# ahuang73/HemoCell

Measured on AMD Instinct MI355X. Metric: MLUPS + cell-vertex updates/s, 256^3 pipeflow 10% Hct, higher is better.
Workload: dtype f64

## Files before the change

### hemocell_amd/capi.py

```python
import ctypes as C
import os
import subprocess

_HERE = os.path.dirname(os.path.abspath(__file__))
LIB_PATH = os.path.join(_HERE, "lib", "libhemocell_amd.so")

c_double_p = C.POINTER(C.c_double)
c_long_p = C.POINTER(C.c_long)
c_int_p = C.POINTER(C.c_int)


class HcError(RuntimeError):
    pass


class Params(C.Structure):
    _fields_ = [(n, C.c_double) for n in
                ("dx", "dt", "nu_p", "rho_p", "kBT_p", "tau", "nu_lbm", "dm", "df", "f_limit", "kBT_lbm")]


class Material(C.Structure):
    _fields_ = [("kLink", C.c_double), ("kArea", C.c_double), ("kVolume", C.c_double), ("kBend", C.c_double),
                ("eta_m", C.c_double), ("radius", C.c_double), ("min_triangles", C.c_int),
                ("aspect_ratio", C.c_double), ("inner_edges", c_long_p), ("n_inner", C.c_int)]
# ... 34 lines not shown
    "hcl_slab_refresh_halos": (C.c_int, [VP, C.c_int]),
    "hcp_slab_sync_placement": (C.c_int, [VP, c_long_p]),
    "hcp_set_envelope": (C.c_int, [VP, C.c_double, c_double_p]),
    "hcp_envelope": (C.c_int, [VP, c_double_p, c_long_p]),
    "hcp_set_deletion_mode": (C.c_int, [VP, C.c_int]),
    "hcp_delete_incomplete_cells": (C.c_int, [VP, c_long_p]),
    "hcp_deletion_counts": (C.c_int, [VP, c_long_p, c_long_p, c_long_p, c_long_p]),
    "hcp_download_alive": (C.c_int, [VP, VP]),
    "hc_profile_enable": (C.c_int, [C.c_int]),
    "hc_profile_read": (C.c_int, [C.c_char_p, c_double_p, c_long_p]),
    "hc_profile_reset": (C.c_int, []),
    "hc_build_tag": (C.c_char_p, []),
    "hc_measure_copy_bandwidth": (C.c_int, [C.c_size_t, C.c_int, c_double_p]),
    "hcl_node_counts": (C.c_int, [VP, c_long_p]),
    "hc_debug_ibm_per_vertex": (C.c_int, [C.c_int]),
    "hc_set_reproducible_spread": (C.c_int, [C.c_int]),
    "hc_debug_force_plane_padding": (C.c_int, [C.c_int]),
    "hcl_create": (C.c_int, [C.POINTER(VP), C.c_int, C.c_int, C.c_int, c_int_p, C.c_double, C.c_int, C.c_int, C.c_int]),
    "hcl_destroy": (C.c_int, [VP]),
    "hcl_set_mask": (C.c_int, [VP, VP]),
    "hcl_init_equilibrium": (C.c_int, [VP, C.c_double, c_double_p]),
    "hcl_set_body_force_regions": (C.c_int, [VP, C.c_int, C.POINTER(C.c_int), c_double_p]),
    "hcl_set_body_force": (C.c_int, [VP, c_double_p]),
    "hcl_set_wall_velocity": (C.c_int, [VP, C.c_int, c_double_p]),
    "hcl_collide_stream": (C.c_int, [VP, C.c_int]),
    "hcl_set_lees_edwards": (C.c_int, [VP, C.c_double, C.c_double]),
    "hcl_set_lees_edwards_displacement": (C.c_int, [VP, C.c_double, C.c_double]),
    "hcl_lees_edwards_apply": (C.c_int, [VP]),
    "hcl_lees_edwards_state": (C.c_int, [VP, c_double_p]),
    "hcl_open_boundary_add": (C.c_int, [VP, C.c_int, C.c_int, c_int_p, C.c_int, c_int_p]),
# ... 165 lines not shown
```

### hemocell_amd/csrc/cells.h

```cpp
#pragma once
#include "common.h"
#include "host_cells.h"
#include "mesh.h"
#include <algorithm>
#include <cmath>
#include <cstring>

using namespace hc;

struct hc_celltype {
  CellTables host;
  DevBuf<int> d_tri, d_edge, d_ebt, d_ebo, d_iedge, d_vtri, d_vtri_k, d_vedge, d_vedge_s, d_bsrc, d_vouter, d_vinner, d_vinner_s, d_ring, d_nring;
  DevBuf<double> d_tri_area_eq, d_edge_len_eq, d_edge_angle_eq, d_patch_eq, d_iedge_len_eq;
};

struct hc_cells {
  hc_lattice *L = nullptr;
  hc_params P;
  int ntypes = 0;
  hc_celltype *types[8];
  int timescale[8];
  HostCells host[8];
  bool host_dirty = false;
  long nverts = 0, cap = 0;
// ... 107 lines not shown
        if (ok) {
          weight = phi2(p[0] - (double)gx) * phi2(p[1] - (double)gy) * phi2(p[2] - (double)gz);
          if (weight != 0.0) {
            node = (lx + HALO) * (long)v.plane + ly * v.nz + lz;
            if (v.mask[node] != 0) node = -1;
          }
        }
        if (node >= 0) total += weight;
        s.node[idx] = node; s.w[idx] = weight; s.lx[idx] = (int)lx; s.ly[idx] = (int)ly; s.lz[idx] = (int)lz;
      }
  const double coeff = 1.0 / total;
#pragma unroll
  for (int idx = 0; idx < 8; idx++) s.w[idx] *= coeff;
}

struct VertArrays { double *p[3], *v[3], *f[3], *r[3]; unsigned char *dead; int *tag; };
struct TypeArrays : VertArrays { const int *vert_cell; int *tag_all; };

template <typename T>
inline int upload_vec(DevBuf<T> &dst, const std::vector<T> &src) {
  const int rc = dst.reserve(src.size() ? src.size() : 1); if (rc != HC_OK) return rc;
  if (src.size()) HC_HIP(hipMemcpy(dst, src.data(), src.size() * sizeof(T), hipMemcpyHostToDevice));
  return HC_OK;
}
template <size_t N>
inline std::vector<int> flatten(const std::vector<std::array<long, N>> &v) {
  std::vector<int> o; o.reserve(v.size() * N);
  for (auto &a : v) for (long x : a) o.push_back((int)x);
  return o;
}
// ... 4 lines not shown
TypeArrays vert_arrays(hc_cells *C, int t);
int ensure_sflag(hc_cells *C);
int solidify_refresh_mask(hc_cells *C);
int solidify_check(hc_cells *C);
const char *solidify_refusal(const hc_lattice *L);
int ensure_rep(hc_cells *C);
int stage_ints(hc_cells *C, int which, int **d, const int *h, int n);
int stage_ints(Staged<int> &s, int **d, const int *h, int n);
int upload_xyz(DevBuf<double> dst[3], long first, const double *src, long n);
int download_xyz(double *dst, const DevBuf<double> src[3], long first, long n);
int append_cells(hc_cells *C, int type, const long *cell_ids, const int *is_new, int n, long n_new);
int interpolate_cells_staged(hc_cells *C, int type, const int *slots, int n, int which);
int wide_spread(hc_cells *C, int type, int force_limit, int per_vertex);
int wide_interpolate(hc_cells *C, int type, const int *slots, int n, int per_vertex);
int wide_emit(hc_cells *C, int type, const int *d_order, long ebase, int force_limit);
inline int ibm_width(const hc_cells *C, int type) { return C->ibm_kernel[type]; }

}
using namespace hcc;
```

### hemocell_amd/csrc/cells.hip

```cpp
#include "cells.h"
#include <cstddef>
#include <memory>
#include <unordered_map>
#include <utility>
#include <vector>

namespace {

__global__ __launch_bounds__(256) void advance_kernel(LatView v, long n, double *px, double *py, double *pz, const double *vx,
                                                      const double *vy, const double *vz, const int *vert_cell, int *tag, unsigned char *dead,
                                                      int *counters, int whole_cell) {
  const long i = (long)blockIdx.x * 256 + threadIdx.x;
  if (i >= n) return;
  const int cell = vert_cell[i];
  if (dead[i] || tag[cell] == 1) return;
  const double x = px[i] + vx[i], y = py[i] + vy[i], z = pz[i] + vz[i];
  px[i] = x; py[i] = y; pz[i] = z;
  long gx = nearest_node(x) - v.x0, gy = nearest_node(y), gz = nearest_node(z);
  bool inside = true;
  if (v.wrap_x) gx = pmod(gx, v.nx); else inside = inside && (gx >= (v.halo_x ? -HALO : 0) && gx < (v.halo_x ? v.nx + HALO : v.nx));
  if (gy < 0 || gy >= v.ny) { if (v.per_y) gy = pmod(gy, v.ny); else inside = false; }
  if (gz < 0 || gz >= v.nz) { if (v.per_z) gz = pmod(gz, v.nz); else inside = false; }
  if (inside && v.mask[(gx + HALO) * (long)v.plane + gy * v.nz + gz] != 0) {
    if (whole_cell) {
      if (atomicExch(&tag[cell], 1) != 1) atomicAdd(&counters[0], 1);
    } else {
      dead[i] = 1;
      atomicAdd(&counters[2], 1);
      if (atomicCAS(&tag[cell], 0, 2) == 0) atomicAdd(&counters[1], 1);
    }
  }
}

__global__ void publish_counters_kernel(const int *counters, int *host_view) { for (int k = 0; k < 4; k++) host_view[k] = counters[k]; }
__global__ void sub_counters_kernel(int *counters, int a, int b, int c, int d) { atomicSub(&counters[0], a); atomicSub(&counters[1], b); atomicSub(&counters[2], c); if (d) atomicSub(&counters[3], d); }

__global__ void delete_incomplete_kernel(long ncells, int *tag, int *counters) {
  const long c = (long)blockIdx.x * 256 + threadIdx.x;
  if (c >= ncells) return;
  if (tag[c] == 2) { tag[c] = 1; atomicAdd(&counters[0], 1); }
}

__global__ void add_vertex_force_kernel(int n, const long *idx, const double *f, double *fx, double *fy, double *fz) {
  const int i = blockIdx.x * 256 + threadIdx.x;
  if (i >= n) return;
  const long v = idx[i];
// ... 668 lines not shown
  if (particles_removed) *particles_removed = C->n_particles_deleted;
  if (incomplete_cells) *incomplete_cells = inc;
  if (missing_particles) *missing_particles = miss;
  return HC_OK;
}

int hcp_download_alive(hc_cells *C, unsigned char *alive) {
  HC_REQUIRE(C && alive, "hcp_download_alive: null pointer");
  int rc = settle(C); if (rc != HC_OK) return rc;
  rc = sync_to_host(C); if (rc != HC_OK) return rc;
  size_t o = 0;
  for (int t = 0; t < C->ntypes; t++) for (unsigned char d : C->host[t].dead) alive[o++] = d ? 0 : 1;
  return HC_OK;
}

int hcp_advance(hc_cells *C, int check_deletions) {
  HC_REQUIRE(C, "hcp_advance: null pointer");
  int rc = sync_to_device(C); if (rc != HC_OK) return rc;
  if (C->nverts == 0) return HC_OK;
  {
    hc::ProfScope prof(hc::PK_ADVANCE);
    const LatView v = make_view(C->L);
    for (int t = 0; t < C->ntypes; t++) {
      const long n = C->ncells[t] * C->types[t]->host.nv;
      if (n == 0) continue;
      const TypeArrays a = vert_arrays(C, t);
      hipLaunchKernelGGL(advance_kernel, dim3((unsigned)((n + 255) / 256)), dim3(256), 0, hc::stream(), v, n, a.p[0], a.p[1], a.p[2], a.v[0], a.v[1], a.v[2],
                         a.vert_cell, a.tag_all, a.dead, C->d_ntag, C->del_mode == HC_DELETE_CELL ? 1 : 0);
      HC_HIP(hipGetLastError());
    }
    C->maybe_tagged = true;
  }
  if (check_deletions) return settle(C);
  return HC_OK;
}

static int g_overlap = 1;
static int g_spread_beside = 1;
int hc_set_overlap(int on) { g_overlap = on != 0; g_spread_beside = on != 2; hcs::set_overlap(on); return HC_OK; }

int hc_iterate(hc_lattice *L, hc_cells *C, long *iter, int n, int particle_timescale, int force_limit, int deletion_check_every) {
  HC_REQUIRE(L && C && iter, "hc_iterate: null pointer");
  HC_REQUIRE(C->L == L, "hc_iterate: cells are bound to a different lattice");
  HC_REQUIRE(particle_timescale >= 1 && deletion_check_every >= 1, "hc_iterate: timescales must be >= 1");
  if (L->n_slabs > 1) return hcs::iterate_slab(L, C, iter, n, particle_timescale, force_limit);
  const bool visc = C->visc_on();
  if (visc) HC_REQUIRE(C->visc_every % particle_timescale == 0 && C->visc_grid_every % particle_timescale == 0,
                       "hc_iterate: the velocity-update timescale must divide both interior-viscosity timescales (hcp_set_interior_timescales)");
  const bool solid = C->solidify_on();
  if (solid) { const char *why = solidify_refusal(L); if (why) { hc::set_error(std::string("hc_iterate: ") + why); return HC_ERR_STATE; } }
// ... 11 lines not shown
      if ((rc = hcp_spread(C, force_limit)) != HC_OK) return rc;
    }
    spread_done = false;
    const bool particle_step = it % particle_timescale == 0;
    const bool visc_grid = visc && it % C->visc_grid_every == 0, visc_membrane = visc && it % C->visc_every == 0;
    const bool solid_check = solid && it % C->solid_every == 0;
    const bool overlap = may_overlap && !particle_step && !visc_grid && !visc_membrane && !solid_check && s + 1 < n;
    if (overlap && (rc = hc::fork()) != HC_OK) return rc;
    if ((rc = hcl_collide_stream_part(L, 0)) != HC_OK) return rc;
    hcl_step_end(L);
    if (L->le_on) {
      if ((rc = hc::lees_edwards_step(L)) != HC_OK) return rc;
      if (L->le_d != 0.0) L->le_D = fmod(L->le_d * (double)(it + 1), (double)L->nx);
    }
    if (L->scalar && (rc = hcl_scalar_step(L->scalar)) != HC_OK) return rc;
    if (particle_step) { if ((rc = hcp_interpolate(C)) != HC_OK) return rc; }
    if (solid_check) { if ((rc = solidify_check(C)) != HC_OK) return rc; }
    if (overlap) hc::route(1);
    if ((rc = hcp_advance(C, 0)) != HC_OK) return rc;
    if ((rc = hcp_mechanics(C, it, 0)) != HC_OK) return rc;
    if (overlap) {
      if (g_spread_beside) { if ((rc = hcp_spread(C, force_limit)) != HC_OK) return rc; spread_done = true; }
      if ((rc = hc::join()) != HC_OK) return rc;
    }
    if (visc_grid) {
      if ((rc = hcp_delete_incomplete_cells(C, nullptr)) != HC_OK) return rc;
      if ((rc = hcp_interior_find(C)) != HC_OK) return rc;
    }
    if (visc_membrane) { if ((rc = hcp_interior_membrane(C)) != HC_OK) return rc; }
    *iter = it + 1;
    if (!overlap && (it + 1) % deletion_check_every == 0 && s + 1 < n) { if ((rc = poll_deletions(C, true)) != HC_OK) return rc; }
  }
  if ((rc = poll_deletions(C, true)) != HC_OK) return rc;
  return solid ? solidify_refresh_mask(C) : HC_OK;
}

}
// ... 1 lines not shown
```

### hemocell_amd/csrc/common.h

```cpp
#pragma once
#include <hip/hip_runtime.h>
#include <stdint.h>
#include <string>
#include <utility>
#include <vector>
#include <type_traits>
#include "../../include/hemocell_amd.h"
#include "d3q19.h"

namespace hc {

void set_error(const std::string &msg);
int hip_fail(hipError_t e, const char *what, const char *file, int line);
hipStream_t stream();
hipStream_t comm_stream();
int fork();
void route(int side);
int join();
bool forked();

#define HC_HIP(call)                                                         \
  do {                                                                       \
    hipError_t e__ = (call);                                                 \
    if (e__ != hipSuccess) return hc::hip_fail(e__, #call, __FILE__, __LINE__); \
// ... 54 lines not shown
  ~Event() { if (e) (void)hipEventDestroy(e); }
  operator hipEvent_t() const { return e; }
  int create() {
    if (e) return HC_OK;
    const hipError_t r = hipEventCreateWithFlags(&e, hipEventDisableTiming);
    if (r != hipSuccess) { e = nullptr; return hip_fail(r, "hipEventCreateWithFlags", __FILE__, __LINE__); }
    return HC_OK;
  }
};
template <class T> struct Staged {
  DevBuf<T> d; PinBuf<T> h; Event ev;
  size_t cap() const { return d.cap < h.cap ? d.cap : h.cap; }
  int reserve(size_t n) { const int rc = d.reserve(n); return rc != HC_OK ? rc : h.reserve(n); }
};

enum ProfKernel { PK_COLLIDE = 0, PK_SPREAD, PK_INTERP, PK_ADVANCE, PK_MECH, PK_COLLIDE_BESIDE, PK_LEES_EDWARDS, PK_COLLIDE_VISC, PK_INTERIOR_FIND, PK_INTERIOR_MEMBRANE, PK_SCALAR, PK_SOLIDIFY_PREPARE, PK_SOLIDIFY_FLAG, PK_COUNT };
void prof_count(int kernel);
struct ProfScope {
  int k; bool on;
  hipEvent_t a, b;
  explicit ProfScope(int kernel);
  ~ProfScope();
};

constexpr int HALO = 2;

constexpr int STAT_BLOCKS = 512;
struct StatAcc { double mn, mx, sum; long n; };
__device__ __forceinline__ void stat_add(StatAcc &a, double v) { a.mn = v < a.mn ? v : a.mn; a.mx = v > a.mx ? v : a.mx; a.sum += v; a.n++; }
__device__ __forceinline__ void stat_block_store(StatAcc a, double *partial ) {
  __shared__ double s_red[4][4];
// ... 167 lines not shown
```

### hemocell_amd/csrc/ibm.hip

```cpp
#include "ibm_common.h"
#include <hipcub/hipcub.hpp>
#include <cstdlib>
#include <cstring>
#include <numeric>

namespace {

__global__ __launch_bounds__(256) void ibm_spread_kernel(LatView v, long n, const double *px, const double *py, const double *pz,
                                                         double *fx, double *fy, double *fz, const double *rx, const double *ry, const double *rz,
                                                         double *F, int limit_on, double f_limit, const int *vert_cell, const int *tag, const unsigned char *dead) {
  const long i = (long)blockIdx.x * 256 + threadIdx.x;
  if (i >= n) return;
  if (dead[i] || tag[vert_cell[i]] == 1) return;
  double f0 = fx[i], f1 = fy[i], f2 = fz[i];
  if (limit_on) {
    const double mag = sqrt((f0 * f0 + f1 * f1) + f2 * f2);
    if (mag > f_limit) {
      const double sc = f_limit / mag;
      f0 *= sc; f1 *= sc; f2 *= sc;
      fx[i] = f0; fy[i] = f1; fz[i] = f2;
    }
  }
  Stencil s;
  phi2_stencil(v, px[i], py[i], pz[i], s);
// ... 170 lines not shown
  if (nb[0] * nb[1] * nb[2] > 64) return false;
  if (threadIdx.x < 64) {
    const int l = threadIdx.x;
    bool near = false;
    if (l < nb[0] * nb[1] * nb[2]) {
      const int bz = l % nb[2], by = (l / nb[2]) % nb[1], bx = l / (nb[2] * nb[1]);
      near = v.wallbrick[((long)(b0[0] + bx) * v.nby + (b0[1] + by)) * v.nbz + (b0[2] + bz)] != 0;
    }
    const unsigned long long any = __ballot(near);
    if (l == 0) *s_near = any != 0ull;
  }
  __syncthreads();
  return *s_near == 0;
}

__device__ __forceinline__ bool cell_prologue(const LatView &v, int nv, long base, const double *px, const double *py, const double *pz,
                                              const unsigned char *dead, int *s_red, int *s_near, unsigned char *mt, Tile &t, VStencil vs[NVPT] PH_PARAM) {
  const int tid = threadIdx.x, nth = blockDim.x;
  double p[NVPT][3]; int b[NVPT][3]; bool live[NVPT];
  int lo[3] = {0x7fffffff, 0x7fffffff, 0x7fffffff}, hi[3] = {-0x7fffffff, -0x7fffffff, -0x7fffffff};
#pragma unroll
  for (int j = 0; j < NVPT; j++) {
    const int i = tid + j * nth;
    live[j] = i < nv && !(dead && dead[base + i]);
    if (live[j]) {
      p[j][0] = px[base + i]; p[j][1] = py[base + i]; p[j][2] = pz[base + i];
      stencil_base(v, p[j][0], p[j][1], p[j][2], b[j]);
#pragma unroll
      for (int a = 0; a < 3; a++) { lo[a] = min(lo[a], b[j][a]); hi[a] = max(hi[a], b[j][a] + 1); }
    }
  }
  block_bbox(lo, hi, s_red, t);
  STAMP(1);
  if (!tile_finish(v, t) || nv > NVPT * nth) return false;
  const bool clear = tile_is_clear(v, t, s_near);
  STAMP(2);
  if (!clear) {
#pragma unroll 4
    for (int i = tid; i < t.vol; i += nth) mt[i] = tile_mask(v, t, i);
    __syncthreads();
  }
  STAMP(3);
#pragma unroll
  for (int j = 0; j < NVPT; j++) {
    vs[j].adm = 0; vs[j].base = 0;
    if (live[j]) tile_stencil(t, clear ? nullptr : mt, p[j][0], p[j][1], p[j][2], b[j], vs[j]);
  }
// ... 17 lines not shown
    const int i = i0 + tid;
    const bool marked = i < t.vol && slot[i] == SLOT_MARK;
    const unsigned long long b = __ballot(marked);
    int first = 0;
    if ((tid & 63) == 0 && b) first = atomicAdd(s_count, (int)__popcll(b));
    first = __shfl(first, 0);
    if (marked) {
      const int n = first + (int)__popcll(b & ((1ull << (tid & 63)) - 1ull));
      if (n < NODE_CAP) { slot[i] = (unsigned short)n; list[n] = (unsigned short)i; }
    }
  }
  __syncthreads();
  return *s_count;
}

__device__ void spread_direct(const LatView &v, int nv, long base, const double *px, const double *py, const double *pz, const double *fx,
                              const double *fy, const double *fz, const double *rx, const double *ry, const double *rz, double *F,
                              const unsigned char *dead) {
  for (int i = threadIdx.x; i < nv; i += blockDim.x) {
    if (dead && dead[base + i]) continue;
    Stencil s;
    phi2_stencil(v, px[base + i], py[base + i], pz[base + i], s);
    const double f0 = (rx ? rx[base + i] : 0.0) + fx[base + i], f1 = (ry ? ry[base + i] : 0.0) + fy[base + i], f2 = (rz ? rz[base + i] : 0.0) + fz[base + i];
#pragma unroll
    for (int k = 0; k < 8; k++) {
      if (s.node[k] < 0) continue;
      v.dirty[s.node[k] >> 4] = v.epoch;
      double *Fn = F + 3 * s.node[k];
      unsafeAtomicAdd(Fn, f0 * s.w[k]);
      unsafeAtomicAdd(Fn + 1, f1 * s.w[k]);
      unsafeAtomicAdd(Fn + 2, f2 * s.w[k]);
    }
  }
}

__global__ __launch_bounds__(256) void ibm_spread_cell_kernel(LatView v, int nv, const double *px, const double *py, const double *pz,
                                                              double *fx, double *fy, double *fz, const double *rx, const double *ry, const double *rz,
                                                              double *F, int limit_on, double f_limit, int xcd_ranges, const int *tag, const unsigned char *vdead) {
  __shared__ unsigned short slot[TILE_CAP];
  __shared__ __attribute__((aligned(16))) unsigned char raw[TILE_CAP > 2 * NODE_CAP ? TILE_CAP : 2 * NODE_CAP];
  unsigned char *mt = raw; unsigned short *list = reinterpret_cast<unsigned short *>(raw);
  __shared__ double acc[3 * NODE_CAP];
  __shared__ int s_red[6 * MAXW], s_count, s_near;
  const int tid = threadIdx.x, nth = blockDim.x;
  PH_INIT
  const int cell = xcd_ranges ? xcd_contiguous((int)blockIdx.x, (int)gridDim.x) : (int)blockIdx.x;
  const int state = tag[cell];
  if (state == 1) return;
  STAMP(0);
  const unsigned char *dead = state == 2 ? vdead : nullptr;
  const long base = (long)cell * nv;
  const bool in_regs = nv <= NVPT * nth;
  double f[NVPT][3];
  if (in_regs) {
#pragma unroll
    for (int j = 0; j < NVPT; j++) {
      const int i = tid + j * nth;
      f[j][0] = f[j][1] = f[j][2] = 0.0;
      if (i < nv) { f[j][0] = fx[base + i]; f[j][1] = fy[base + i]; f[j][2] = fz[base + i]; }
    }
  }
  Tile t; VStencil vs[NVPT];
  bool tiled = cell_prologue(v, nv, base, px, py, pz, dead, s_red, &s_near, mt, t, vs PH_ARG);
  if (limit_on) {
    if (in_regs) {
#pragma unroll
      for (int j = 0; j < NVPT; j++) {
        const int i = tid + j * nth;
        if (i < nv && !(dead && dead[base + i])) {
          const double mag = sqrt((f[j][0] * f[j][0] + f[j][1] * f[j][1]) + f[j][2] * f[j][2]);
          if (mag > f_limit) { const double sc = f_limit / mag; f[j][0] *= sc; f[j][1] *= sc; f[j][2] *= sc; fx[base + i] = f[j][0]; fy[base + i] = f[j][1]; fz[base + i] = f[j][2]; }
        }
      }
    } else {
      for (int i = tid; i < nv; i += nth) {
        if (dead && dead[base + i]) continue;
        const double f0 = fx[base + i], f1 = fy[base + i], f2 = fz[base + i];
        const double mag = sqrt((f0 * f0 + f1 * f1) + f2 * f2);
// ... 21 lines not shown
    }
  }
  __syncthreads();
  STAMP(6);
  for (int k = tid; k < 3 * n; k += nth) {
    const double val = acc[k];
    if (val != 0.0) {
      const int q = k / 3;
      int lx, ly, lz; const long node = tile_node(v, t, list[q], lx, ly, lz); v.dirty[node >> 4] = v.epoch;
      unsafeAtomicAdd(&F[3 * node + (k - 3 * q)], val);
    }
  }
  STAMP(7);
}

template <bool OPEN = false>
__global__ __launch_bounds__(256) void ibm_interpolate_cell_kernel(LatView v, Pops<OPEN> pv, int nv, const double *px, const double *py,
                                                                   const double *pz, double *vx, double *vy, double *vz, const int *slots, int xcd_ranges,
                                                                   const int *tag, const unsigned char *vdead) {
  __shared__ unsigned short slot[TILE_CAP];
  __shared__ __attribute__((aligned(16))) unsigned char raw[TILE_CAP > 2 * NODE_CAP ? TILE_CAP : 2 * NODE_CAP];
  unsigned char *mt = raw; unsigned short *list = reinterpret_cast<unsigned short *>(raw);
  __shared__ double ux[NODE_CAP], uy[NODE_CAP], uz[NODE_CAP];
  __shared__ int s_red[6 * MAXW], s_count, s_near;
  const int tid = threadIdx.x, nth = blockDim.x;
  const int cell = slots ? slots[blockIdx.x] : (xcd_ranges ? xcd_contiguous((int)blockIdx.x, (int)gridDim.x) : (int)blockIdx.x);
  const int state = tag[cell];
  if (state == 1) return;
  const unsigned char *dead = state == 2 ? vdead : nullptr;
  const long base = (long)cell * nv;
  Tile t; VStencil vs[NVPT];
  PH_INIT
  bool tiled = cell_prologue(v, nv, base, px, py, pz, dead, s_red, &s_near, mt, t, vs PH_ARG);
  const int sy = t.e[2], sx = t.e[1] * t.e[2];
  if (tiled) {
    if (compact_nodes(t, vs, slot, list, &s_count) > NODE_CAP) tiled = false;
    STAMP(12);
  }
  if (tiled) {
    const int n = s_count;
    for (int k = tid; k < n; k += nth) {
      int lx, ly, lz;
      const long node = tile_node(v, t, list[k], lx, ly, lz);
      double u[3];
      node_velocity<OPEN>(v, pv, lx, ly, lz, node, u);
      ux[k] = u[0]; uy[k] = u[1]; uz[k] = u[2];
    }
    __syncthreads();
    STAMP(13);
#pragma unroll
    for (int j = 0; j < NVPT; j++) {
      const int i = tid + j * nth;
      if (i >= nv || (dead && dead[base + i])) continue;
      double a0 = 0.0, a1 = 0.0, a2 = 0.0;
#pragma unroll
      for (int k = 0; k < 8; k++) {
        if (!(vs[j].adm & (1u << k))) continue;
        const int q = slot[vs[j].base + (k >> 2) * sx + ((k >> 1) & 1) * sy + (k & 1)];
        a0 += (ux[q] * vs[j].w[k]); a1 += (uy[q] * vs[j].w[k]); a2 += (uz[q] * vs[j].w[k]);
      }
      vx[base + i] = a0; vy[base + i] = a1; vz[base + i] = a2;
    }
    STAMP(14);
    return;
  }
  for (int i = tid; i < nv; i += nth) {
    if (dead && dead[base + i]) continue;
    Stencil s;
    phi2_stencil(v, px[base + i], py[base + i], pz[base + i], s);
    double a0 = 0.0, a1 = 0.0, a2 = 0.0;
#pragma unroll
    for (int k = 0; k < 8; k++) {
      if (s.node[k] < 0) continue;
      double u[3];
      node_velocity<OPEN>(v, pv, s.lx[k], s.ly[k], s.lz[k], s.node[k], u);
      a0 += (u[0] * s.w[k]); a1 += (u[1] * s.w[k]); a2 += (u[2] * s.w[k]);
    }
    vx[base + i] = a0; vy[base + i] = a1; vz[base + i] = a2;
  }
}


}

static int g_ibm_per_vertex = 0;
extern "C" int hc_debug_ibm_per_vertex(int on) { g_ibm_per_vertex = on; return HC_OK; }
static int g_reproducible = -1;
static bool reproducible() {
  if (g_reproducible < 0) { const char *e = std::getenv("HEMOCELL_REPRODUCIBLE_SPREAD"); g_reproducible = (e && *e && *e != '0') ? 1 : 0; }
  return g_reproducible == 1;
}
extern "C" int hc_set_reproducible_spread(int on) { g_reproducible = on ? 1 : 0; return HC_OK; }

static int spread_reproducible(hc_cells *C, int force_limit) {
  const LatView v = make_view(C->L);
  long n_e = 0, first_e[8];
  for (int t = 0; t < C->ntypes; t++) {
    const long w = ibm_width(C, t);
    first_e[t] = n_e;
    n_e += (C->ncells[t] * C->types[t]->host.nv * w * w * w + 7) / 8 * 8;
  }
  HC_REQUIRE(v.npad * 3 < 0xffffffffL && n_e < 0x7fffffffL, "reproducible spread: lattice or vertex count beyond its 32-bit keys");
  int rc;
  if (n_e > C->det_cap) {
    HC_HIP(hipDeviceSynchronize());
    const long cap = n_e + n_e / 4 + 4096;
    C->det_cap = 0;
// ... 39 lines not shown
  return HC_OK;
}
#ifdef HC_IBM_PHASE_TIMES
extern "C" int hc_debug_phase_times(double *out) {
  unsigned long long h[32];
  if (hipMemcpyFromSymbol(h, HIP_SYMBOL(g_phase), sizeof(h)) != hipSuccess) return HC_ERR_HIP;
  for (int k = 0; k < 32; k++) out[k] = (double)h[k];
  std::memset(h, 0, sizeof(h));
  if (hipMemcpyToSymbol(HIP_SYMBOL(g_phase), h, sizeof(h)) != hipSuccess) return HC_ERR_HIP;
  return HC_OK;
}
#endif

extern "C" {

int hcp_spread(hc_cells *C, int force_limit) {
  HC_REQUIRE(C, "hcp_spread: null pointer");
  int rc = sync_to_device(C); if (rc != HC_OK) return rc;
  if (C->nverts == 0) return HC_OK;
  hc::ProfScope prof(hc::PK_SPREAD);
  if (reproducible()) return spread_reproducible(C, force_limit);
  const LatView v = make_view(C->L);
  for (int t = 0; t < C->ntypes; t++) {
    const long n = C->ncells[t] * C->types[t]->host.nv;
    if (n == 0) continue;
    const int nv = C->types[t]->host.nv;
    if (ibm_width(C, t) != HC_IBM_PHI2) { if ((rc = wide_spread(C, t, force_limit, g_ibm_per_vertex)) != HC_OK) return rc; continue; }
    const TypeArrays a = vert_arrays(C, t);
    if (g_ibm_per_vertex)
      hipLaunchKernelGGL(ibm_spread_kernel, dim3((unsigned)((n + 255) / 256)), dim3(256), 0, hc::stream(), v, n, a.p[0], a.p[1], a.p[2], a.f[0], a.f[1], a.f[2],
                         a.r[0], a.r[1], a.r[2], C->L->force[C->L->fcur], force_limit, C->P.f_limit, a.vert_cell, a.tag_all, a.dead);
    else
      hipLaunchKernelGGL(ibm_spread_cell_kernel, dim3((unsigned)C->ncells[t]), dim3(nv > 128 ? 256 : 128), 0, hc::stream(), v, nv, a.p[0], a.p[1], a.p[2],
                         a.f[0], a.f[1], a.f[2], a.r[0], a.r[1], a.r[2], C->L->force[C->L->fcur], force_limit, C->P.f_limit, 1, a.tag, a.dead);
    HC_HIP(hipGetLastError());
  }
  return HC_OK;
}

int hcp_interpolate(hc_cells *C) {
  HC_REQUIRE(C, "hcp_interpolate: null pointer");
  int rc = sync_to_device(C); if (rc != HC_OK) return rc;
  if (C->nverts == 0) return HC_OK;
  hc::ProfScope prof(hc::PK_INTERP);
  const hc_lattice *L = C->L;
  const LatView v = make_view(L);
  const PopView pv = make_pops(L);
  for (int t = 0; t < C->ntypes; t++) {
    const long n = C->ncells[t] * C->types[t]->host.nv;
    if (n == 0) continue;
    const int nv = C->types[t]->host.nv;
    if (ibm_width(C, t) != HC_IBM_PHI2) { if ((rc = wide_interpolate(C, t, nullptr, 0, g_ibm_per_vertex)) != HC_OK) return rc; continue; }
    const TypeArrays a = vert_arrays(C, t);
    if (g_ibm_per_vertex)
      HC_LAUNCH_POPS(ibm_interpolate_kernel, dim3((unsigned)((n + 255) / 256)), dim3(256), v, pv, n, a.p[0], a.p[1], a.p[2], a.v[0], a.v[1], a.v[2],
                     a.vert_cell, a.tag_all, a.dead);
    else
      HC_LAUNCH_POPS(ibm_interpolate_cell_kernel, dim3((unsigned)C->ncells[t]), dim3(nv > 128 ? 256 : 128), v, pv, nv, a.p[0], a.p[1], a.p[2], a.v[0], a.v[1], a.v[2],
                     (const int *)nullptr, 1, a.tag, a.dead);
    HC_HIP(hipGetLastError());
  }
  return HC_OK;
}

int hcl_face_velocity_pack(hc_lattice *L, int side, double *dev_buf) {
  HC_REQUIRE(L && dev_buf && (side == 0 || side == 1), "hcl_face_velocity_pack: bad arguments");
  LatView v = make_view(L);
  v.halo_u[0] = v.halo_u[1] = nullptr;
  const PopView pv = make_pops(L);
  HC_LAUNCH_POPS(face_velocity_kernel, dim3((unsigned)((L->plane + 255) / 256), 1, 1), dim3(256), v, pv, side == 0 ? 0 : L->nx - 1, dev_buf, 0, (double *)nullptr);
  HC_HIP(hipGetLastError());
  return HC_OK;
}
int hcl_face_velocity_pack_both(hc_lattice *L, double *dev_lo, double *dev_hi) {
  HC_REQUIRE(L, "hcl_face_velocity_pack_both: null lattice");
  if (!dev_lo && !dev_hi) return HC_OK;
  if (!dev_lo || !dev_hi) return hcl_face_velocity_pack(L, dev_lo ? 0 : 1, dev_lo ? dev_lo : dev_hi);
  LatView v = make_view(L);
// ... 22 lines not shown
  HC_REQUIRE(C && type >= 0 && type < C->ntypes && n >= 0 && which >= 0 && which < 19, "hcp_interpolate_cells: bad arguments");
  if (n == 0) return HC_OK;
  HC_REQUIRE(slots, "hcp_interpolate_cells: null pointer");
  int rc = sync_to_device(C); if (rc != HC_OK) return rc;
  for (int i = 0; i < n; i++) HC_REQUIRE(slots[i] >= 0 && slots[i] < C->ncells[type], "hcp_interpolate_cells: slot out of range");
  int *d_slots = nullptr;
  rc = stage_ints(C, which, &d_slots, slots, n); if (rc != HC_OK) return rc;
  hc::ProfScope prof(hc::PK_INTERP);
  if (ibm_width(C, type) != HC_IBM_PHI2) return wide_interpolate(C, type, d_slots, n, 0);
  const hc_lattice *L = C->L;
  const LatView v = make_view(L);
  const PopView pv = make_pops(L);
  const TypeArrays a = vert_arrays(C, type);
  const int nv = C->types[type]->host.nv;
  HC_LAUNCH_POPS(ibm_interpolate_cell_kernel, dim3((unsigned)n), dim3(nv > 128 ? 256 : 128), v, pv, nv, a.p[0], a.p[1], a.p[2], a.v[0], a.v[1], a.v[2],
                 (const int *)d_slots, 0, a.tag, a.dead);
  HC_HIP(hipGetLastError());
  return HC_OK;
}
```

### hemocell_amd/csrc/runtime.hip

```cpp
#include "common.h"
#include <cstdlib>
#include <cstring>
#include <mutex>

namespace hc {

static thread_local std::string g_error;
static hipStream_t g_own_stream = nullptr;
static hipStream_t g_stream = nullptr;
static hipStream_t g_side = nullptr;
static hipStream_t g_comm = nullptr;
static hipEvent_t g_fork_ev = nullptr, g_join_ev = nullptr;
static bool g_on_side = false, g_forked = false;
static bool g_initialised = false;
static bool g_profile = false;

struct ProfRecord { hipEvent_t a, b; };
static std::vector<ProfRecord> g_prof[PK_COUNT];
static double g_prof_ms[PK_COUNT];
static long g_prof_n[PK_COUNT];

void set_error(const std::string &msg) { g_error = msg; }
int hip_fail(hipError_t e, const char *what, const char *file, int line) {
  g_error = std::string("HIP error ") + hipGetErrorName(e) + " (" + hipGetErrorString(e) + ") in " + what + " at " + file + ":" + std::to_string(line);
// ... 147 lines not shown
  if (e0) hipEventDestroy(e0);
  if (e1) hipEventDestroy(e1);
  if (e != hipSuccess) return hc::hip_fail(e, "hc_measure_copy_bandwidth", __FILE__, __LINE__);
  *gbytes_per_s = 2.0 * (double)bytes * repeats / ((double)ms * 1e-3) / 1e9;
  return HC_OK;
}

int hc_profile_enable(int on) { hc::g_profile = on != 0; return HC_OK; }
int hc_profile_reset(void) {
  hc::prof_collect();
  for (int k = 0; k < hc::PK_COUNT; k++) { hc::g_prof_ms[k] = 0; hc::g_prof_n[k] = 0; }
  return HC_OK;
}
int hc_profile_read(const char *kernel, double *total_ms, long *launches) {
  HC_REQUIRE(kernel && total_ms && launches, "hc_profile_read: null pointer");
  static const char *names[hc::PK_COUNT] = {"collide_stream_alone", "ibm_spread", "ibm_interpolate", "advance", "mechanics", "collide_stream_beside", "lees_edwards", "collide_stream_interior", "interior_find", "interior_membrane", "scalar_step", "solidify_prepare", "solidify_flag"};
  hc::prof_collect();
  if (std::strcmp(kernel, "collide_stream") == 0) {
    *total_ms = hc::g_prof_ms[hc::PK_COLLIDE] + hc::g_prof_ms[hc::PK_COLLIDE_BESIDE];
    *launches = hc::g_prof_n[hc::PK_COLLIDE] + hc::g_prof_n[hc::PK_COLLIDE_BESIDE];
    return HC_OK;
  }
  for (int k = 0; k < hc::PK_COUNT; k++)
    if (std::strcmp(kernel, names[k]) == 0) { *total_ms = hc::g_prof_ms[k]; *launches = hc::g_prof_n[k]; return HC_OK; }
  hc::set_error(std::string("hc_profile_read: unknown kernel ") + kernel);
  return HC_ERR_ARG;
}

}
```

### include/hemocell_amd.h

```cpp
#ifndef HEMOCELL_AMD_H
#define HEMOCELL_AMD_H

#include <stddef.h>
#include <stdint.h>

#ifdef __cplusplus
extern "C" {
#endif

#define HC_OK 0
#define HC_ERR_HIP 1
#define HC_ERR_ARG 2
#define HC_ERR_STATE 3

#define HC_Q 19

typedef struct hc_lattice hc_lattice;
typedef struct hc_celltype hc_celltype;
typedef struct hc_cells hc_cells;

const char *hc_last_error(void);
int hc_init(int device);
int hc_device_count(int *count);
int hc_set_stream(void *hip_stream);
int hc_synchronize(void);
int hc_fork(void);
int hc_route(int side);
int hc_join(void);
int hc_side_stream(void **hip_stream);
int hc_set_overlap(int on);
int hc_profile_enable(int on);
int hc_profile_read(const char *kernel, double *total_ms, long *launches);
int hc_profile_reset(void);
const char *hc_build_tag(void);
int hc_measure_copy_bandwidth(size_t bytes, int repeats, double *gbytes_per_s);
int hc_set_reproducible_spread(int on);
int hc_debug_ibm_per_vertex(int on);
int hc_debug_force_plane_padding(int on);

#define HC_TRANSPORT_NONE 0
#define HC_TRANSPORT_RCCL 1
#define HC_TRANSPORT_TCP 2
#define HC_TRANSPORT_AUTO 3
int hc_comm_init_env(void);
int hc_comm_init(int rank, int world, int local_rank, const char *master_addr, int port, int transport, int init_device);
int hc_comm_finalize(void);
int hc_comm_info(int *rank, int *world, int *transport);
int hc_comm_barrier(void);
int hc_comm_allreduce(double *v, int n, int op);
int hc_comm_bcast(void *buf, size_t bytes, int root);
int hc_comm_allgather(const void *mine, size_t bytes, void *all);
int hc_comm_exchange_host(int periodic, const void *send_lo, size_t n_lo, const void *send_hi, size_t n_hi,
// ... 228 lines not shown
```

Baseline: 15710.

## Fuse vertex advance into per-cell IBM interpolate and spread kernels

Folds the position-advance and boundary-deletion test into the per-cell interpolation kernel on particle steps, and into the per-cell spread kernel on substeps where only spreading runs. The separate advance kernel is skipped for the fused types. This removes one launch and one full re-read and write of vertex position and velocity arrays per step. In exchange, the cell kernels get more registers and branches, and the spread and advance ordering now depends on a debug mask and the timescale logic.

```diff
diff --git a/hemocell_amd/capi.py b/hemocell_amd/capi.py
--- a/hemocell_amd/capi.py
+++ b/hemocell_amd/capi.py
@@ -72,6 +72,7 @@
     "hc_measure_copy_bandwidth": (C.c_int, [C.c_size_t, C.c_int, c_double_p]),
     "hcl_node_counts": (C.c_int, [VP, c_long_p]),
     "hc_debug_ibm_per_vertex": (C.c_int, [C.c_int]),
+    "hc_debug_fused_vertex_path": (C.c_int, [C.c_int]),
     "hc_set_reproducible_spread": (C.c_int, [C.c_int]),
     "hc_debug_force_plane_padding": (C.c_int, [C.c_int]),
     "hcl_create": (C.c_int, [C.POINTER(VP), C.c_int, C.c_int, C.c_int, c_int_p, C.c_double, C.c_int, C.c_int, C.c_int]),
diff --git a/hemocell_amd/csrc/cells.h b/hemocell_amd/csrc/cells.h
--- a/hemocell_amd/csrc/cells.h
+++ b/hemocell_amd/csrc/cells.h
@@ -145,6 +145,24 @@
   for (int idx = 0; idx < 8; idx++) s.w[idx] *= coeff;
 }
 
+__device__ __forceinline__ bool advance_boundary_test(const LatView &v, double x, double y, double z, int *tag_cell, unsigned char *dead_i,
+                                                      int *counters, int whole_cell) {
+  long gx = nearest_node(x) - v.x0, gy = nearest_node(y), gz = nearest_node(z);
+  bool inside = true;
+  if (v.wrap_x) gx = pmod(gx, v.nx); else inside = inside && (gx >= (v.halo_x ? -HALO : 0) && gx < (v.halo_x ? v.nx + HALO : v.nx));
+  if (gy < 0 || gy >= v.ny) { if (v.per_y) gy = pmod(gy, v.ny); else inside = false; }
+  if (gz < 0 || gz >= v.nz) { if (v.per_z) gz = pmod(gz, v.nz); else inside = false; }
+  if (!(inside && v.mask[(gx + HALO) * (long)v.plane + gy * v.nz + gz] != 0)) return false;
+  if (whole_cell) {
+    if (atomicExch(tag_cell, 1) != 1) atomicAdd(&counters[0], 1);
+  } else {
+    *dead_i = 1;
+    atomicAdd(&counters[2], 1);
+    if (atomicCAS(tag_cell, 0, 2) == 0) atomicAdd(&counters[1], 1);
+  }
+  return true;
+}
+
 struct VertArrays { double *p[3], *v[3], *f[3], *r[3]; unsigned char *dead; int *tag; };
 struct TypeArrays : VertArrays { const int *vert_cell; int *tag_all; };
 
@@ -179,6 +197,9 @@
 int wide_spread(hc_cells *C, int type, int force_limit, int per_vertex);
 int wide_interpolate(hc_cells *C, int type, const int *slots, int n, int per_vertex);
 int wide_emit(hc_cells *C, int type, const int *d_order, long ebase, int force_limit);
+unsigned fused_types(const hc_cells *C, int bit);
+int interpolate_fused(hc_cells *C, unsigned advance);
+int spread_fused(hc_cells *C, int force_limit, unsigned advance);
 inline int ibm_width(const hc_cells *C, int type) { return C->ibm_kernel[type]; }
 
 }
diff --git a/hemocell_amd/csrc/cells.hip b/hemocell_amd/csrc/cells.hip
--- a/hemocell_amd/csrc/cells.hip
+++ b/hemocell_amd/csrc/cells.hip
@@ -16,20 +16,7 @@
   if (dead[i] || tag[cell] == 1) return;
   const double x = px[i] + vx[i], y = py[i] + vy[i], z = pz[i] + vz[i];
   px[i] = x; py[i] = y; pz[i] = z;
-  long gx = nearest_node(x) - v.x0, gy = nearest_node(y), gz = nearest_node(z);
-  bool inside = true;
-  if (v.wrap_x) gx = pmod(gx, v.nx); else inside = inside && (gx >= (v.halo_x ? -HALO : 0) && gx < (v.halo_x ? v.nx + HALO : v.nx));
-  if (gy < 0 || gy >= v.ny) { if (v.per_y) gy = pmod(gy, v.ny); else inside = false; }
-  if (gz < 0 || gz >= v.nz) { if (v.per_z) gz = pmod(gz, v.nz); else inside = false; }
-  if (inside && v.mask[(gx + HALO) * (long)v.plane + gy * v.nz + gz] != 0) {
-    if (whole_cell) {
-      if (atomicExch(&tag[cell], 1) != 1) atomicAdd(&counters[0], 1);
-    } else {
-      dead[i] = 1;
-      atomicAdd(&counters[2], 1);
-      if (atomicCAS(&tag[cell], 0, 2) == 0) atomicAdd(&counters[1], 1);
-    }
-  }
+  advance_boundary_test(v, x, y, z, &tag[cell], &dead[i], counters, whole_cell);
 }
 
 __global__ void publish_counters_kernel(const int *counters, int *host_view) { for (int k = 0; k < 4; k++) host_view[k] = counters[k]; }
@@ -728,26 +715,32 @@
   return HC_OK;
 }
 
-int hcp_advance(hc_cells *C, int check_deletions) {
+static int advance_types(hc_cells *C, int check_deletions, unsigned skip) {
   HC_REQUIRE(C, "hcp_advance: null pointer");
   int rc = sync_to_device(C); if (rc != HC_OK) return rc;
   if (C->nverts == 0) return HC_OK;
-  {
+  bool any = false;
+  for (int t = 0; t < C->ntypes; t++) any = any || (C->ncells[t] > 0 && !(skip >> t & 1u));
+  if (any) {
     hc::ProfScope prof(hc::PK_ADVANCE);
     const LatView v = make_view(C->L);
     for (int t = 0; t < C->ntypes; t++) {
       const long n = C->ncells[t] * C->types[t]->host.nv;
-      if (n == 0) continue;
+      if (n == 0 || (skip >> t & 1u)) continue;
       const TypeArrays a = vert_arrays(C, t);
       hipLaunchKernelGGL(advance_kernel, dim3((unsigned)((n + 255) / 256)), dim3(256), 0, hc::stream(), v, n, a.p[0], a.p[1], a.p[2], a.v[0], a.v[1], a.v[2],
                          a.vert_cell, a.tag_all, a.dead, C->d_ntag, C->del_mode == HC_DELETE_CELL ? 1 : 0);
       HC_HIP(hipGetLastError());
     }
     C->maybe_tagged = true;
+  } else {
+    hc::prof_count(hc::PK_ADVANCE);
   }
   if (check_deletions) return settle(C);
   return HC_OK;
 }
+
+int hcp_advance(hc_cells *C, int check_deletions) { return advance_types(C, check_deletions, 0u); }
 
 static int g_overlap = 1;
 static int g_spread_beside = 1;
@@ -789,13 +782,20 @@
       if (L->le_d != 0.0) L->le_D = fmod(L->le_d * (double)(it + 1), (double)L->nx);
     }
     if (L->scalar && (rc = hcl_scalar_step(L->scalar)) != HC_OK) return rc;
-    if (particle_step) { if ((rc = hcp_interpolate(C)) != HC_OK) return rc; }
+    unsigned in_interp = 0, in_spread = 0;
+    if (particle_step && !solid_check) in_interp = fused_types(C, 0);
+    if (overlap && g_spread_beside) {
+      in_spread = fused_types(C, 1);
+      for (int t = 0; t < C->ntypes; t++) if (it % C->timescale[t] == 0) in_spread &= ~(1u << t);
+    }
+    if (in_interp | in_spread) hc::prof_count(hc::PK_ADVANCE_FUSED);
+    if (particle_step) { if ((rc = interpolate_fused(C, in_interp)) != HC_OK) return rc; }
     if (solid_check) { if ((rc = solidify_check(C)) != HC_OK) return rc; }
     if (overlap) hc::route(1);
-    if ((rc = hcp_advance(C, 0)) != HC_OK) return rc;
+    if ((rc = advance_types(C, 0, in_interp | in_spread)) != HC_OK) return rc;
     if ((rc = hcp_mechanics(C, it, 0)) != HC_OK) return rc;
     if (overlap) {
-      if (g_spread_beside) { if ((rc = hcp_spread(C, force_limit)) != HC_OK) return rc; spread_done = true; }
+      if (g_spread_beside) { if ((rc = spread_fused(C, force_limit, in_spread)) != HC_OK) return rc; spread_done = true; }
       if ((rc = hc::join()) != HC_OK) return rc;
     }
     if (visc_grid) {
diff --git a/hemocell_amd/csrc/common.h b/hemocell_amd/csrc/common.h
--- a/hemocell_amd/csrc/common.h
+++ b/hemocell_amd/csrc/common.h
@@ -92,7 +92,7 @@
   int reserve(size_t n) { const int rc = d.reserve(n); return rc != HC_OK ? rc : h.reserve(n); }
 };
 
-enum ProfKernel { PK_COLLIDE = 0, PK_SPREAD, PK_INTERP, PK_ADVANCE, PK_MECH, PK_COLLIDE_BESIDE, PK_LEES_EDWARDS, PK_COLLIDE_VISC, PK_INTERIOR_FIND, PK_INTERIOR_MEMBRANE, PK_SCALAR, PK_SOLIDIFY_PREPARE, PK_SOLIDIFY_FLAG, PK_COUNT };
+enum ProfKernel { PK_COLLIDE = 0, PK_SPREAD, PK_INTERP, PK_ADVANCE, PK_MECH, PK_COLLIDE_BESIDE, PK_LEES_EDWARDS, PK_COLLIDE_VISC, PK_INTERIOR_FIND, PK_INTERIOR_MEMBRANE, PK_SCALAR, PK_SOLIDIFY_PREPARE, PK_SOLIDIFY_FLAG, PK_ADVANCE_FUSED, PK_COUNT };
 void prof_count(int kernel);
 struct ProfScope {
   int k; bool on;
diff --git a/hemocell_amd/csrc/ibm.hip b/hemocell_amd/csrc/ibm.hip
--- a/hemocell_amd/csrc/ibm.hip
+++ b/hemocell_amd/csrc/ibm.hip
@@ -208,23 +208,50 @@
   return *s_near == 0;
 }
 
-__device__ __forceinline__ bool cell_prologue(const LatView &v, int nv, long base, const double *px, const double *py, const double *pz,
-                                              const unsigned char *dead, int *s_red, int *s_near, unsigned char *mt, Tile &t, VStencil vs[NVPT] PH_PARAM) {
+struct AdvanceArgs { const double *vx, *vy, *vz; int *tag_cell; unsigned char *vdead; int *counters; int whole_cell; };
+
+template <bool ADVANCE> using PosPtr = std::conditional_t<ADVANCE, double *, const double *>;
+template <bool ADVANCE> using TagPtr = std::conditional_t<ADVANCE, int *, const int *>;
+template <bool ADVANCE> using DeadPtr = std::conditional_t<ADVANCE, unsigned char *, const unsigned char *>;
+
+template <bool ADVANCE = false>
+__device__ __forceinline__ bool cell_prologue(const LatView &v, int nv, long base, PosPtr<ADVANCE> px, PosPtr<ADVANCE> py, PosPtr<ADVANCE> pz,
+                                             const unsigned char *dead, int *s_red, int *s_near, unsigned char *mt, Tile &t, VStencil vs[NVPT],
+                                             double p[NVPT][3], const AdvanceArgs *adv, int *s_gone, bool *gone_out PH_PARAM) {
   const int tid = threadIdx.x, nth = blockDim.x;
-  double p[NVPT][3]; int b[NVPT][3]; bool live[NVPT];
+  int b[NVPT][3]; bool live[NVPT];
   int lo[3] = {0x7fffffff, 0x7fffffff, 0x7fffffff}, hi[3] = {-0x7fffffff, -0x7fffffff, -0x7fffffff};
+  [[maybe_unused]] bool hit = false;
 #pragma unroll
   for (int j = 0; j < NVPT; j++) {
     const int i = tid + j * nth;
     live[j] = i < nv && !(dead && dead[base + i]);
     if (live[j]) {
       p[j][0] = px[base + i]; p[j][1] = py[base + i]; p[j][2] = pz[base + i];
+      if constexpr (ADVANCE) {
+        p[j][0] = p[j][0] + adv->vx[base + i]; p[j][1] = p[j][1] + adv->vy[base + i]; p[j][2] = p[j][2] + adv->vz[base + i];
+        px[base + i] = p[j][0]; py[base + i] = p[j][1]; pz[base + i] = p[j][2];
+        if (advance_boundary_test(v, p[j][0], p[j][1], p[j][2], adv->tag_cell, adv->vdead + base + i, adv->counters, adv->whole_cell)) {
+          hit = true; live[j] = false;
+        }
+      }
+    }
+    if (live[j]) {
       stencil_base(v, p[j][0], p[j][1], p[j][2], b[j]);
 #pragma unroll
       for (int a = 0; a < 3; a++) { lo[a] = min(lo[a], b[j][a]); hi[a] = max(hi[a], b[j][a] + 1); }
     }
   }
+  if constexpr (ADVANCE) {
+    const unsigned long long any = __ballot(hit && adv->whole_cell);
+    if ((tid & 63) == 0) s_gone[tid >> 6] = any != 0ull;
+  }
   block_bbox(lo, hi, s_red, t);
+  if constexpr (ADVANCE) {
+    int gone = 0;
+    for (int w = 0; w < (nth + 63) >> 6; w++) gone |= s_gone[w];
+    if (gone) { *gone_out = true; return false; }
+  }
   STAMP(1);
   if (!tile_finish(v, t) || nv > NVPT * nth) return false;
   const bool clear = tile_is_clear(v, t, s_near);
@@ -272,6 +299,23 @@
   return *s_count;
 }
 
+__device__ bool advance_direct(const LatView &v, int nv, long base, double *px, double *py, double *pz, const unsigned char *dead,
+                               const AdvanceArgs &adv, int *s_gone) {
+  bool hit = false;
+  for (int i = threadIdx.x; i < nv; i += blockDim.x) {
+    if (dead[base + i]) continue;
+    const double x = px[base + i] + adv.vx[base + i], y = py[base + i] + adv.vy[base + i], z = pz[base + i] + adv.vz[base + i];
+    px[base + i] = x; py[base + i] = y; pz[base + i] = z;
+    hit = advance_boundary_test(v, x, y, z, adv.tag_cell, adv.vdead + base + i, adv.counters, adv.whole_cell) || hit;
+  }
+  const unsigned long long any = __ballot(hit && adv.whole_cell);
+  if ((threadIdx.x & 63) == 0) s_gone[threadIdx.x >> 6] = any != 0ull;
+  __syncthreads();
+  int gone = 0;
+  for (int w = 0; w < (int)((blockDim.x + 63) >> 6); w++) gone |= s_gone[w];
+  return gone != 0;
+}
+
 __device__ void spread_direct(const LatView &v, int nv, long base, const double *px, const double *py, const double *pz, const double *fx,
                               const double *fy, const double *fz, const double *rx, const double *ry, const double *rz, double *F,
                               const unsigned char *dead) {
@@ -292,21 +336,24 @@
   }
 }
 
-__global__ __launch_bounds__(256) void ibm_spread_cell_kernel(LatView v, int nv, const double *px, const double *py, const double *pz,
+template <bool ADVANCE = false>
+__global__ __launch_bounds__(256) void ibm_spread_cell_kernel(LatView v, int nv, PosPtr<ADVANCE> px, PosPtr<ADVANCE> py, PosPtr<ADVANCE> pz,
                                                               double *fx, double *fy, double *fz, const double *rx, const double *ry, const double *rz,
-                                                              double *F, int limit_on, double f_limit, int xcd_ranges, const int *tag, const unsigned char *vdead) {
+                                                              double *F, int limit_on, double f_limit, int xcd_ranges, TagPtr<ADVANCE> tag, DeadPtr<ADVANCE> vdead,
+                                                              const double *avx, const double *avy, const double *avz, int *counters, int whole_cell) {
   __shared__ unsigned short slot[TILE_CAP];
   __shared__ __attribute__((aligned(16))) unsigned char raw[TILE_CAP > 2 * NODE_CAP ? TILE_CAP : 2 * NODE_CAP];
   unsigned char *mt = raw; unsigned short *list = reinterpret_cast<unsigned short *>(raw);
   __shared__ double acc[3 * NODE_CAP];
   __shared__ int s_red[6 * MAXW], s_count, s_near;
+  __shared__ int s_gone[ADVANCE ? MAXW : 1];
   const int tid = threadIdx.x, nth = blockDim.x;
   PH_INIT
   const int cell = xcd_ranges ? xcd_contiguous((int)blockIdx.x, (int)gridDim.x) : (int)blockIdx.x;
   const int state = tag[cell];
   if (state == 1) return;
   STAMP(0);
-  const unsigned char *dead = state == 2 ? vdead : nullptr;
+  const unsigned char *dead = (ADVANCE || state == 2) ? vdead : nullptr;
   const long base = (long)cell * nv;
   const bool in_regs = nv <= NVPT * nth;
   double f[NVPT][3];
@@ -318,8 +365,21 @@
       if (i < nv) { f[j][0] = fx[base + i]; f[j][1] = fy[base + i]; f[j][2] = fz[base + i]; }
     }
   }
-  Tile t; VStencil vs[NVPT];
-  bool tiled = cell_prologue(v, nv, base, px, py, pz, dead, s_red, &s_near, mt, t, vs PH_ARG);
+  Tile t; VStencil vs[NVPT]; double p[NVPT][3];
+  bool tiled;
+  if constexpr (ADVANCE) {
+    const AdvanceArgs adv{avx, avy, avz, &tag[cell], vdead, counters, whole_cell};
+    if (!in_regs) {
+      if (advance_direct(v, nv, base, px, py, pz, dead, adv, s_gone)) return;
+      tiled = false;
+    } else {
+      bool gone = false;
+      tiled = cell_prologue<true>(v, nv, base, px, py, pz, dead, s_red, &s_near, mt, t, vs, p, &adv, s_gone, &gone PH_ARG);
+      if (gone) return;
+    }
+  } else {
+    tiled = cell_prologue(v, nv, base, px, py, pz, dead, s_red, &s_near, mt, t, vs, p, nullptr, nullptr, nullptr PH_ARG);
+  }
   if (limit_on) {
     if (in_regs) {
 #pragma unroll
@@ -371,10 +431,10 @@
   STAMP(7);
 }
 
-template <bool OPEN = false>
-__global__ __launch_bounds__(256) void ibm_interpolate_cell_kernel(LatView v, Pops<OPEN> pv, int nv, const double *px, const double *py,
-                                                                   const double *pz, double *vx, double *vy, double *vz, const int *slots, int xcd_ranges,
-                                                                   const int *tag, const unsigned char *vdead) {
+template <bool OPEN = false, bool ADVANCE = false>
+__global__ __launch_bounds__(256) void ibm_interpolate_cell_kernel(LatView v, Pops<OPEN> pv, int nv, PosPtr<ADVANCE> px, PosPtr<ADVANCE> py,
+                                                                   PosPtr<ADVANCE> pz, double *vx, double *vy, double *vz, const int *slots, int xcd_ranges,
+                                                                   TagPtr<ADVANCE> tag, DeadPtr<ADVANCE> vdead, int *counters, int whole_cell) {
   __shared__ unsigned short slot[TILE_CAP];
   __shared__ __attribute__((aligned(16))) unsigned char raw[TILE_CAP > 2 * NODE_CAP ? TILE_CAP : 2 * NODE_CAP];
   unsigned char *mt = raw; unsigned short *list = reinterpret_cast<unsigned short *>(raw);
@@ -386,9 +446,9 @@
   if (state == 1) return;
   const unsigned char *dead = state == 2 ? vdead : nullptr;
   const long base = (long)cell * nv;
-  Tile t; VStencil vs[NVPT];
+  Tile t; VStencil vs[NVPT]; double p[NVPT][3];
   PH_INIT
-  bool tiled = cell_prologue(v, nv, base, px, py, pz, dead, s_red, &s_near, mt, t, vs PH_ARG);
+  bool tiled = cell_prologue(v, nv, base, px, py, pz, dead, s_red, &s_near, mt, t, vs, p, nullptr, nullptr, nullptr PH_ARG);
   const int sy = t.e[2], sx = t.e[1] * t.e[2];
   if (tiled) {
     if (compact_nodes(t, vs, slot, list, &s_count) > NODE_CAP) tiled = false;
@@ -417,6 +477,11 @@
         a0 += (ux[q] * vs[j].w[k]); a1 += (uy[q] * vs[j].w[k]); a2 += (uz[q] * vs[j].w[k]);
       }
       vx[base + i] = a0; vy[base + i] = a1; vz[base + i] = a2;
+      if constexpr (ADVANCE) {
+        const double x = p[j][0] + a0, y = p[j][1] + a1, z = p[j][2] + a2;
+        px[base + i] = x; py[base + i] = y; pz[base + i] = z;
+        advance_boundary_test(v, x, y, z, &tag[cell], vdead + base + i, counters, whole_cell);
+      }
     }
     STAMP(14);
     return;
@@ -434,6 +499,11 @@
       a0 += (u[0] * s.w[k]); a1 += (u[1] * s.w[k]); a2 += (u[2] * s.w[k]);
     }
     vx[base + i] = a0; vy[base + i] = a1; vz[base + i] = a2;
+    if constexpr (ADVANCE) {
+      const double x = px[base + i] + a0, y = py[base + i] + a1, z = pz[base + i] + a2;
+      px[base + i] = x; py[base + i] = y; pz[base + i] = z;
+      advance_boundary_test(v, x, y, z, &tag[cell], vdead + base + i, counters, whole_cell);
+    }
   }
 }
 
@@ -448,6 +518,14 @@
   return g_reproducible == 1;
 }
 extern "C" int hc_set_reproducible_spread(int on) { g_reproducible = on ? 1 : 0; return HC_OK; }
+static int g_fused_vertex_path = 7;
+extern "C" int hc_debug_fused_vertex_path(int mask) { g_fused_vertex_path = mask & 7; return HC_OK; }
+unsigned hcc::fused_types(const hc_cells *C, int bit) {
+  if (!(g_fused_vertex_path >> bit & 1) || g_ibm_per_vertex || (bit == 1 && reproducible())) return 0u;
+  unsigned m = 0;
+  for (int t = 0; t < C->ntypes; t++) if (ibm_width(C, t) == HC_IBM_PHI2 && C->ncells[t] > 0) m |= 1u << t;
+  return m;
+}
 
 static int spread_reproducible(hc_cells *C, int force_limit) {
   const LatView v = make_view(C->L);
@@ -517,32 +595,46 @@
 
 extern "C" {
 
-int hcp_spread(hc_cells *C, int force_limit) {
+int hcp_spread(hc_cells *C, int force_limit) { return hcc::spread_fused(C, force_limit, 0u); }
+int hcp_interpolate(hc_cells *C) { return hcc::interpolate_fused(C, 0u); }
+
+}
+
+int hcc::spread_fused(hc_cells *C, int force_limit, unsigned advance) {
   HC_REQUIRE(C, "hcp_spread: null pointer");
   int rc = sync_to_device(C); if (rc != HC_OK) return rc;
   if (C->nverts == 0) return HC_OK;
   hc::ProfScope prof(hc::PK_SPREAD);
+  HC_REQUIRE(!advance || (!reproducible() && !g_ibm_per_vertex), "hcp_spread: only the atomic per-cell spread advances");
   if (reproducible()) return spread_reproducible(C, force_limit);
   const LatView v = make_view(C->L);
+  if (advance) C->maybe_tagged = true;
   for (int t = 0; t < C->ntypes; t++) {
     const long n = C->ncells[t] * C->types[t]->host.nv;
     if (n == 0) continue;
     const int nv = C->types[t]->host.nv;
+    const dim3 block = dim3(nv > 128 ? 256 : 128);
     if (ibm_width(C, t) != HC_IBM_PHI2) { if ((rc = wide_spread(C, t, force_limit, g_ibm_per_vertex)) != HC_OK) return rc; continue; }
     const TypeArrays a = vert_arrays(C, t);
     if (g_ibm_per_vertex)
       hipLaunchKernelGGL(ibm_spread_kernel, dim3((unsigned)((n + 255) / 256)), dim3(256), 0, hc::stream(), v, n, a.p[0], a.p[1], a.p[2], a.f[0], a.f[1], a.f[2],
                          a.r[0], a.r[1], a.r[2], C->L->force[C->L->fcur], force_limit, C->P.f_limit, a.vert_cell, a.tag_all, a.dead);
+    else if (advance >> t & 1u)
+      hipLaunchKernelGGL(ibm_spread_cell_kernel<true>, dim3((unsigned)C->ncells[t]), block, 0, hc::stream(), v, nv, a.p[0], a.p[1], a.p[2],
+                         a.f[0], a.f[1], a.f[2], a.r[0], a.r[1], a.r[2], C->L->force[C->L->fcur], force_limit, C->P.f_limit, 1, a.tag, a.dead,
+                         a.v[0], a.v[1], a.v[2], (int *)C->d_ntag, C->del_mode == HC_DELETE_CELL ? 1 : 0);
     else
-      hipLaunchKernelGGL(ibm_spread_cell_kernel, dim3((unsigned)C->ncells[t]), dim3(nv > 128 ? 256 : 128), 0, hc::stream(), v, nv, a.p[0], a.p[1], a.p[2],
-                         a.f[0], a.f[1], a.f[2], a.r[0], a.r[1], a.r[2], C->L->force[C->L->fcur], force_limit, C->P.f_limit, 1, a.tag, a.dead);
+      hipLaunchKernelGGL(ibm_spread_cell_kernel<false>, dim3((unsigned)C->ncells[t]), block, 0, hc::stream(), v, nv, a.p[0], a.p[1], a.p[2],
+                         a.f[0], a.f[1], a.f[2], a.r[0], a.r[1], a.r[2], C->L->force[C->L->fcur], force_limit, C->P.f_limit, 1, a.tag, a.dead,
+                         (const double *)nullptr, (const double *)nullptr, (const double *)nullptr, (int *)nullptr, 0);
     HC_HIP(hipGetLastError());
   }
   return HC_OK;
 }
 
-int hcp_interpolate(hc_cells *C) {
+int hcc::interpolate_fused(hc_cells *C, unsigned advance) {
   HC_REQUIRE(C, "hcp_interpolate: null pointer");
+  HC_REQUIRE(!advance || !g_ibm_per_vertex, "hcp_interpolate: only the per-cell interpolation advances");
   int rc = sync_to_device(C); if (rc != HC_OK) return rc;
   if (C->nverts == 0) return HC_OK;
   hc::ProfScope prof(hc::PK_INTERP);
@@ -553,18 +645,28 @@
     const long n = C->ncells[t] * C->types[t]->host.nv;
     if (n == 0) continue;
     const int nv = C->types[t]->host.nv;
+    const dim3 block = dim3(nv > 128 ? 256 : 128);
     if (ibm_width(C, t) != HC_IBM_PHI2) { if ((rc = wide_interpolate(C, t, nullptr, 0, g_ibm_per_vertex)) != HC_OK) return rc; continue; }
     const TypeArrays a = vert_arrays(C, t);
     if (g_ibm_per_vertex)
       HC_LAUNCH_POPS(ibm_interpolate_kernel, dim3((unsigned)((n + 255) / 256)), dim3(256), v, pv, n, a.p[0], a.p[1], a.p[2], a.v[0], a.v[1], a.v[2],
                      a.vert_cell, a.tag_all, a.dead);
-    else
-      HC_LAUNCH_POPS(ibm_interpolate_cell_kernel, dim3((unsigned)C->ncells[t]), dim3(nv > 128 ? 256 : 128), v, pv, nv, a.p[0], a.p[1], a.p[2], a.v[0], a.v[1], a.v[2],
-                     (const int *)nullptr, 1, a.tag, a.dead);
+    else if (advance >> t & 1u) {
+      hc::launch_open(L, pv, [&](auto open, const auto &pops) {
+        hipLaunchKernelGGL((ibm_interpolate_cell_kernel<decltype(open)::value, true>), dim3((unsigned)C->ncells[t]), block, 0, hc::stream(), v, pops,
+                           nv, a.p[0], a.p[1], a.p[2], a.v[0], a.v[1], a.v[2], (const int *)nullptr, 1, a.tag, a.dead, (int *)C->d_ntag,
+                           C->del_mode == HC_DELETE_CELL ? 1 : 0);
+      });
+      C->maybe_tagged = true;
+    } else
+      HC_LAUNCH_POPS(ibm_interpolate_cell_kernel, dim3((unsigned)C->ncells[t]), block, v, pv, nv, a.p[0], a.p[1], a.p[2], a.v[0], a.v[1], a.v[2],
+                     (const int *)nullptr, 1, a.tag, a.dead, (int *)nullptr, 0);
     HC_HIP(hipGetLastError());
   }
   return HC_OK;
 }
+
+extern "C" {
 
 int hcl_face_velocity_pack(hc_lattice *L, int side, double *dev_buf) {
   HC_REQUIRE(L && dev_buf && (side == 0 || side == 1), "hcl_face_velocity_pack: bad arguments");
@@ -617,7 +719,7 @@
   const TypeArrays a = vert_arrays(C, type);
   const int nv = C->types[type]->host.nv;
   HC_LAUNCH_POPS(ibm_interpolate_cell_kernel, dim3((unsigned)n), dim3(nv > 128 ? 256 : 128), v, pv, nv, a.p[0], a.p[1], a.p[2], a.v[0], a.v[1], a.v[2],
-                 (const int *)d_slots, 0, a.tag, a.dead);
+                 (const int *)d_slots, 0, a.tag, a.dead, (int *)nullptr, 0);
   HC_HIP(hipGetLastError());
   return HC_OK;
 }
diff --git a/hemocell_amd/csrc/runtime.hip b/hemocell_amd/csrc/runtime.hip
--- a/hemocell_amd/csrc/runtime.hip
+++ b/hemocell_amd/csrc/runtime.hip
@@ -185,7 +185,7 @@
 }
 int hc_profile_read(const char *kernel, double *total_ms, long *launches) {
   HC_REQUIRE(kernel && total_ms && launches, "hc_profile_read: null pointer");
-  static const char *names[hc::PK_COUNT] = {"collide_stream_alone", "ibm_spread", "ibm_interpolate", "advance", "mechanics", "collide_stream_beside", "lees_edwards", "collide_stream_interior", "interior_find", "interior_membrane", "scalar_step", "solidify_prepare", "solidify_flag"};
+  static const char *names[hc::PK_COUNT] = {"collide_stream_alone", "ibm_spread", "ibm_interpolate", "advance", "mechanics", "collide_stream_beside", "lees_edwards", "collide_stream_interior", "interior_find", "interior_membrane", "scalar_step", "solidify_prepare", "solidify_flag", "advance_fused"};
   hc::prof_collect();
   if (std::strcmp(kernel, "collide_stream") == 0) {
     *total_ms = hc::g_prof_ms[hc::PK_COLLIDE] + hc::g_prof_ms[hc::PK_COLLIDE_BESIDE];
diff --git a/include/hemocell_amd.h b/include/hemocell_amd.h
--- a/include/hemocell_amd.h
+++ b/include/hemocell_amd.h
@@ -36,6 +36,7 @@
 int hc_measure_copy_bandwidth(size_t bytes, int repeats, double *gbytes_per_s);
 int hc_set_reproducible_spread(int on);
 int hc_debug_ibm_per_vertex(int on);
+int hc_debug_fused_vertex_path(int mask);
 int hc_debug_force_plane_padding(int on);
 
 #define HC_TRANSPORT_NONE 0
```

After: 15890 (median of 6 runs). +1.2%, better.
